# nanoporetech/pomfret

Measured on AMD Instinct MI355X. Metric: aligned reads/sec (methphase kernel), higher is better.
Workload: dtype u32/f32

## Files before the change

### pomfret_amd/csrc/pf_kernels.hip

```cpp
#include <hip/hip_runtime.h>
#include <stdint.h>
#include "pf_device.h"

#define DEV static __device__ __forceinline__

#ifdef PF_K3_PROFILE
DEV unsigned long long k3_stamp_now() {
    unsigned long long t;
    __builtin_amdgcn_sched_barrier(0);
    asm volatile("s_memtime %0\n\ts_waitcnt lgkmcnt(0)" : "=s"(t) :: "memory");
    __builtin_amdgcn_sched_barrier(0);
    return t;
}
#define K3_STAMP(i) do { const unsigned long long t_ = k3_stamp_now(); \
    prof_acc[i] += t_ - prof_last; prof_last = t_; } while (0)
DEV unsigned long long k3_realtime() {
    unsigned long long t;
    asm volatile("s_memrealtime %0\n\ts_waitcnt lgkmcnt(0)" : "=s"(t) :: "memory");
    return t;
}
#define K3_COUNT(i, v) do { prof_acc[i] += (v); } while (0)
#define K12_STAMP(i) do { if (threadIdx.x == 0) { const unsigned long long t_ = k3_stamp_now(); \
    d.prof[64ull * d.W + (uint64_t)w * 16 + (i)] = t_ - k12_t0; k12_t0 = t_; } } while (0)
#define K2_STAMP(i) do { if (k2acc) { const unsigned long long t_ = k3_stamp_now(); \
// ... 134 lines not shown
DEV double swap32_add_d(double x) {
    const long long b = __double_as_longlong(x);
    const auto lo = __builtin_amdgcn_permlane32_swap((uint32_t)b, (uint32_t)b, false, false);
    const auto hi = __builtin_amdgcn_permlane32_swap((uint32_t)(b >> 32), (uint32_t)(b >> 32), false, false);
    const double a = __longlong_as_double((long long)(((uint64_t)hi[0] << 32) | lo[0]));
    const double c = __longlong_as_double((long long)(((uint64_t)hi[1] << 32) | lo[1]));
    return a + c;
}
DEV double wave_group_sum_d(double x, uint32_t ncp) {
    if (ncp < 2) x = ror_add_d<1>(x);
    if (ncp < 4) x = ror_add_d<2>(x);
    if (ncp < 8) x = ror_add_d<4>(x);
    if (ncp < 16) x = ror_add_d<8>(x);
    if (ncp < 32) x = swap16_add_d(x);
    if (ncp < 64) x = swap32_add_d(x);
    return x;
}

DEV uint32_t rdl(uint32_t x, uint32_t l) { return (uint32_t)__builtin_amdgcn_readlane((int)x, (int)l); }

DEV uint64_t wave_max_u64(uint64_t x) {
#pragma unroll
    for (int o = 32; o > 0; o >>= 1) {
        uint64_t y = __shfl_xor(x, o, 64);
        x = y > x ? y : x;
    }
    return x;
}

template <int NT>
DEV uint32_t block_excl_scan(uint32_t v, uint32_t *sh, uint32_t *total) {
    const uint32_t tid = threadIdx.x, lane = tid & 63, wid = tid >> 6;
    constexpr int NW = NT / 64;
    uint32_t x = wave_incl_scan(v, lane);
    if (lane == 63) sh[wid] = x;
    __syncthreads();
    if (wid == 0) {
        uint32_t t = lane < (uint32_t)NW ? sh[lane] : 0;
        uint32_t s = wave_incl_scan(t, lane);
        if (lane < (uint32_t)NW) sh[lane] = s - t;
        if (lane == NW - 1) sh[NW] = s;
    }
    __syncthreads();
    uint32_t res = x - v + sh[wid];
    *total = sh[NW];
    __syncthreads();
    return res;
}

DEV uint64_t lb_u32(const uint32_t *a, uint64_t lo, uint64_t hi, uint32_t v) {
    while (lo < hi) {
        uint64_t mid = lo + ((hi - lo) >> 1);
        if (a[mid] < v) lo = mid + 1; else hi = mid;
    }
    return lo;
}
DEV uint64_t ub_u32(const uint32_t *a, uint64_t lo, uint64_t hi, uint32_t v) {
    while (lo < hi) {
        uint64_t mid = lo + ((hi - lo) >> 1);
        if (a[mid] <= v) lo = mid + 1; else hi = mid;
    }
    return lo;
}

DEV uint32_t next_pow2(uint32_t x) { return x <= 1 ? 1u : 1u << (32 - __clz(x - 1)); }


DEV void k2_chars(const pf_dev_batch &d, uint64_t c0, uint64_t c1, const uint32_t *sp, uint32_t qlo,
                  uint32_t qhi, uint32_t lane, uint8_t *chars) {
    const uint32_t nq = qhi - qlo;
    for (uint32_t j = lane; j < nq; j += 64) chars[j] = 2;
    wave_sync();
    const uint32_t plo = sp[qlo], phi = sp[qhi - 1];
    for (uint64_t cb = c0 + lane; cb < c1; cb += 256) {
        uint32_t pos[4], prv[4], cat[4];
#pragma unroll
        for (int u = 0; u < 4; u++) {
            const uint64_t c = cb + 64 * u;
            const bool ok = c < c1;
            pos[u] = ok ? d.call_pos[c] : 0xFFFFFFFFu;
            prv[u] = (ok && c > c0) ? d.call_pos[c - 1] : 0xFFFFFFFFu;
            cat[u] = ok ? d.call_cat[c] : 2u;
        }
#pragma unroll
        for (int u = 0; u < 4; u++) {
            const uint64_t c = cb + 64 * u;
            const uint32_t p = pos[u];
            if (c < c1 && (c == c0 || prv[u] != p) && p >= plo && p <= phi) {
                uint32_t lo = qlo, hi = qhi;
                while (lo < hi) {
                    const uint32_t mid = (lo + hi) >> 1;
                    if (sp[mid] < p) lo = mid + 1; else hi = mid;
                }
                if (lo < qhi && sp[lo] == p) chars[lo - qlo] = (uint8_t)cat[u];
            }
        }
    }
    wave_sync();
}

DEV void wave_lb2(const uint32_t *a, uint32_t n, uint32_t kA, uint32_t kB, uint32_t lane, uint32_t &lbA,
                  uint32_t &lbB) {
    const uint32_t h = lane >> 5, j = lane & 31;
    const uint32_t key = h ? kB : kA;
    uint32_t lo = 0, hi = n;
    for (;;) {
        const uint32_t len = hi - lo;
        const uint32_t step = (len + 31) >> 5;
        const uint32_t p = lo + j * step;
        const bool lt = len > 0 && p < hi && a[p] < key;
        const uint64_t bal = __ballot(lt);
        const uint32_t c = (uint32_t)__popc((uint32_t)(bal >> (32 * h)));
        if (len > 0) {
            if (c == 0) hi = lo;
            else {
                const uint32_t pn = lo + c * step;
                lo = lo + (c - 1) * step + 1;
                hi = pn < hi ? pn : hi;
            }
        }
        if (__ballot(hi > lo) == 0) break;
    }
    lbA = rdl(lo, 0);
    lbB = rdl(lo, 32);
}

struct K2SiteHash {
    const uint32_t *t;
    uint32_t mask, pmin;
};
DEV uint32_t k2_hash_slot(uint32_t rel) { return (rel * 2654435761u) >> 7; }
DEV uint32_t k2_site_of(const K2SiteHash &hs, uint32_t p) {
    const uint32_t rel = p - hs.pmin;
    if (p < hs.pmin || rel >= (1u << 19)) return PF_NONE;
    uint32_t h = k2_hash_slot(rel) & hs.mask;
    for (;;) {
        const uint32_t e = hs.t[h];
        if (e == PF_NONE) return PF_NONE;
        if ((e >> 13) == rel) return e & 8191u;
        h = (h + 1) & hs.mask;
    }
}

struct K2Read {
    uint64_t c0, c1;
    uint32_t F, L, cap, maxcall;
};

#define K2_CR 8
struct K2Calls {
    uint32_t pos[K2_CR], cat[K2_CR], site[K2_CR];
};

DEV void k2_calls_sites(K2Calls &cl, const uint32_t *sp, uint32_t S, const K2SiteHash hs, bool use_hash) {
#pragma unroll
    for (int u = 0; u < K2_CR; u++) {
        const uint32_t p = cl.pos[u];
        uint32_t si = PF_NONE;
        if (cl.cat[u] < 3u && S > 0 && p >= sp[0] && p <= sp[S - 1]) {
            if (use_hash) si = k2_site_of(hs, p);
            else {
                uint32_t lo = 0, hi = S;
                while (lo < hi) {
                    const uint32_t mid = (lo + hi) >> 1;
                    if (sp[mid] < p) lo = mid + 1; else hi = mid;
                }
                si = sp[lo] == p ? lo : PF_NONE;
            }
        }
        cl.site[u] = si;
    }
}

DEV void k2_load_scalars(const pf_dev_batch &d, uint32_t r, K2Read &rd) {
    rd.c0 = d.read_call_off[r];
    rd.c1 = d.read_call_end[r];
    rd.F = d.read_first[r];
    rd.L = d.read_last[r];
    rd.cap = d.mmr_cap[r];
    rd.maxcall = 0;
}

DEV void k2_issue_calls(const pf_dev_batch &d, const K2Read &rd, uint32_t lane, uint32_t *pos, uint32_t *cat) {
    const bool fits = rd.c1 - rd.c0 <= 64ull * K2_CR && rd.cap <= d.k12_capw;
#pragma unroll
    for (int u = 0; u < K2_CR; u++) {
        const uint64_t c = rd.c0 + lane + 64u * u;
        const bool ok = fits && c < rd.c1;
        pos[u] = ok ? d.call_pos[c] : 0xFFFFFFFFu;
        cat[u] = ok ? (uint32_t)d.call_cat[c] : 3u;
    }
}

DEV void k2_finish_calls(uint64_t c0, uint64_t c1, uint32_t lane, const uint32_t *pos, const uint32_t *cat,
                         K2Calls &cl) {
    uint32_t last = 0xFFFFFFFFu;
#pragma unroll
    for (int u = 0; u < K2_CR; u++) {
        const uint64_t c = c0 + lane + 64u * u;
        uint32_t prv = (uint32_t)__builtin_amdgcn_update_dpp(0, (int)pos[u], 0x138, 0xF, 0xF, false);
        if (lane == 0) prv = last;
        last = rdl(pos[u], 63);
        cl.pos[u] = pos[u];
        cl.cat[u] = (c < c1 && (c == c0 || prv != pos[u])) ? cat[u] : 3u;
    }
}

DEV void k2_chars_reg(const K2Calls &cl, uint32_t qlo, uint32_t qhi, uint32_t lane, uint8_t *chars) {
    const uint32_t nq = qhi - qlo;
    for (uint32_t j = lane; j < nq; j += 64) chars[j] = 2;
    wave_sync();
#pragma unroll
    for (int u = 0; u < K2_CR; u++) {
        const uint32_t si = cl.site[u];
        if (si >= qlo && si < qhi) chars[si - qlo] = (uint8_t)cl.cat[u];
    }
    wave_sync();
}

template <typename IR>
DEV uint32_t k2_core(const pf_dev_batch &d, uint32_t r, uint32_t dir, uint32_t lane, uint32_t S,
                     const uint32_t *sp, const uint32_t *st, const uint8_t *lens, const uint32_t *q1,
                     uint8_t *chars, uint8_t *crank, IR *irank, uint32_t capw, const K2Read &rd,
                     const K2Calls *cl, uint64_t koff, unsigned long long *k2acc = nullptr,
                     uint32_t *kst = nullptr) {
    uint32_t staged_n = 0;
    const uint32_t g = 2 * r + dir;
    const uint64_t c0 = rd.c0, c1 = rd.c1;
    uint32_t total = 0, start_i = PF_NONE;
    if (S > 0 && c1 > c0) {
        const uint32_t F = rd.F, L = rd.L;
        const uint32_t sfirst = st[0], slast = st[S - 1];
        if (!(F > slast || L < sfirst)) {
            uint32_t lbF, lbL;
            wave_lb2(st, S, F, L, lane, lbF, lbL);
            uint32_t xl, xr;
            if (F < sfirst) xl = 0;
            else xl = st[lbF] == F ? lbF : (lbF ? lbF - 1 : 0);
            xr = L > slast ? S : lbL;
            if (xl < xr) {
                const uint32_t qlo = dir ? q1[xl] : xl;
                const uint32_t qhi = dir ? q1[xr - 1] + 1 : xr;
                const uint32_t nq = qhi - qlo;
                const uint32_t cap = rd.cap;
                if (nq > capw || xr - xl > capw) {
                    if (lane == 0) atomicOr(d.status, PF_ST_INTERNAL);
                } else {
                    K2_STAMP(0);
                    if (cl) k2_chars_reg(*cl, qlo, qhi, lane, chars);
                    else k2_chars(d, c0, c1, sp, qlo, qhi, lane, chars);
                    K2_STAMP(1);
                    uint32_t E = 0;
                    for (uint32_t i0 = xl; i0 < xr; i0 += 64) {
                        const uint32_t i = i0 + lane;
                        bool ent = false;
                        if (i < xr) ent = !(i > 1 && st[i] == st[i - 1]);
                        const uint64_t m = __ballot(ent);
                        if (ent) {
                            const uint32_t rk = E + (uint32_t)__popcll(m & lanemask_lt(lane));
                            const uint32_t q = dir ? q1[i] : i;
                            crank[rk] = chars[q - qlo];
                            irank[rk] = (IR)i;
                        }
                        E += (uint32_t)__popcll(m);
                    }
                    wave_sync();
                    K2_STAMP(2);
                    if (E > 0) {
                        const uint32_t maxcall = rd.maxcall;
                        const uint32_t usable = E - (st[irank[E - 1]] > maxcall ? 1u : 0u);
                        if (lane == 0 && E >= 2 && irank[0] == 0 && irank[1] == 1 && st[1] == st[0])
                            crank[0] = 2;
                        wave_sync();
                        uint32_t *out = d.keys + koff;
                        const uint64_t room = d.keys_cap > koff ? d.keys_cap - koff : 0;
                        for (uint32_t e0 = 0; e0 < E; e0 += 64) {
                            const uint32_t e = e0 + lane;
                            uint32_t ne = 0, fj = PF_NONE, i = 0, P = 0;
                            if (e < E) {
                                i = irank[e];
                                P = st[i];
                                for (uint32_t j = i; j < S && st[j] == P; j++) {
                                    if (e + lens[j] <= usable) {
                                        if (fj == PF_NONE) fj = j;
                                        ne++;
                                    }
                                }
                            }
                            const uint32_t incl = wave_incl_scan_dpp(ne);
                            const uint32_t tot = rdl(incl, 63);
                            if (start_i == PF_NONE && tot > 0) {
                                const uint64_t m = __ballot(ne > 0);
                                const uint32_t src = (uint32_t)__ffsll((unsigned long long)m) - 1;
                                start_i = rdl(fj, src);
                            }
                            if (ne) {
                                uint32_t pos = total + incl - ne;
                                for (uint32_t j = i; j < S && st[j] == P; j++) {
                                    const uint32_t Lj = lens[j];
                                    if (e + Lj <= usable) {
                                        uint32_t key = 0;
                                        for (uint32_t t = 0; t < Lj; t++) key = key << 2 | crank[e + t];
                                        if (pos < cap && pos < room) {
                                            if (kst) kst[pos] = key;
                                            else out[pos] = key;
                                        }
                                        pos++;
                                    }
                                }
                            }
                            total += tot;
                        }
                        if (total > cap && lane == 0) atomicOr(d.status, PF_ST_KEYS_OVF);
                        staged_n = total < cap ? total : cap;
                        staged_n = staged_n < room ? staged_n : (uint32_t)room;
                        K2_STAMP(3);
                    }
                }
            }
        }
    }
    if (lane == 0) {
        d.mmr_n[g] = total;
        d.mmr_start[g] = total ? start_i : 0;
    }
    return staged_n;
}

DEV void k2_flush(const pf_dev_batch &d, const uint32_t *kst, uint64_t koff, uint32_t n, uint32_t lane) {
    uint32_t *out = d.keys + koff;
    for (uint32_t t = lane; t < n; t += 64) out[t] = kst[t];
}

__global__ __launch_bounds__(PF_K2_WAVES * 64) void pf_k2_methmers(pf_dev_batch d) {
    __shared__ uint8_t s_chars[PF_K2_WAVES][PF_K2_ENT_CAP];
    __shared__ uint8_t s_crank[PF_K2_WAVES][PF_K2_ENT_CAP];
    __shared__ uint32_t s_irank[PF_K2_WAVES][PF_K2_ENT_CAP];
    const uint32_t lane = threadIdx.x & 63, wid = threadIdx.x >> 6;
    const uint64_t n = 2ull * (*d.fb_ctr);
    for (uint64_t gw = (uint64_t)blockIdx.x * PF_K2_WAVES + wid; gw < n; gw += (uint64_t)gridDim.x * PF_K2_WAVES) {
        const uint32_t r = d.fb_list[gw >> 1], dir = (uint32_t)(gw & 1);
        const uint32_t w = d.read_win[r];
        const uint32_t S = d.win_S[w];
        const uint64_t sb = d.win_site_off[w];
        const uint32_t *sp = d.site_pos + sb;
        const uint32_t *st = dir ? d.st1_pos + sb : sp;
        const uint8_t *lens = (dir ? d.len1 : d.len0) + sb;
        const uint32_t *q1 = d.site_q1 + sb;
        const uint64_t bo = d.big_off[r];
        K2Read rd;
        rd.c0 = d.read_call_off[r];
        rd.c1 = d.read_call_end[r];
        rd.F = d.read_first[r];
        rd.L = d.read_last[r];
        rd.cap = d.mmr_cap[r];
        rd.maxcall = rd.c1 > rd.c0 ? d.call_pos[rd.c1 - 1] : 0u;
        const uint64_t koff = d.mmr_off[2ull * r + dir];
        if (bo == ~0ull) {
            k2_core(d, r, dir, lane, S, sp, st, lens, q1, s_chars[wid], s_crank[wid], s_irank[wid],
                    PF_K2_ENT_CAP, rd, nullptr, koff);
        } else {
            const uint32_t cap = d.mmr_cap[r];
            if (bo + 16ull * cap > d.big_cap) {
                if (lane == 0) { d.mmr_n[2 * r + dir] = 0; d.mmr_start[2 * r + dir] = 0; atomicOr(d.status, PF_ST_BIG_OVF); }
                continue;
            }
            uint8_t *b = d.big + bo + (dir ? 8ull * cap : 0);
            k2_core(d, r, dir, lane, S, sp, st, lens, q1, b, b + cap, reinterpret_cast<uint32_t *>(b + 4ull * cap),
                    cap, rd, nullptr, koff);
        }
    }
}

DEV void k12_methmers(const pf_dev_batch &d, uint32_t r0, uint32_t i0, uint32_t i1, uint32_t wid, uint32_t NW,
                      uint32_t lane, uint32_t S, const uint32_t *sp, const uint32_t *st1, const uint32_t *q1s,
                      const uint8_t *l0s, const uint8_t *l1s, const K2SiteHash &hsd, bool use_hash, uint8_t *wb,
                      unsigned long long *k2acc, uint32_t *rctr) {
        uint8_t *chars = wb, *crank = wb + PF_K12_CAPW;
        uint16_t *irank = reinterpret_cast<uint16_t *>(wb + 2 * PF_K12_CAPW);
        uint32_t *kst = reinterpret_cast<uint32_t *>(wb + 4 * PF_K12_CAPW);
        uint32_t pend_n = 0;
        uint64_t pend_off = 0;
        auto take = [&]() -> uint32_t {
            uint32_t v = 0;
            if (lane == 0) v = atomicAdd(rctr, 1u);
            return (uint32_t)__builtin_amdgcn_readfirstlane((int)v);
        };
        K2Read rdA, rdB;
        uint32_t pA[K2_CR], tA[K2_CR], pB[K2_CR], tB[K2_CR];
        const uint32_t iw = i0 + wid;
        uint32_t iB = iw < i1 ? take() : i1;
        if (iw < i1) k2_load_scalars(d, r0 + iw, rdA);
        if (iB < i1) k2_load_scalars(d, r0 + iB, rdB);
        k2_issue_calls(d, iw < i1 ? rdA : K2Read{0, 0, 0, 0, 0, 0}, lane, pA, tA);
        for (uint32_t i = iw; i < i1;) {
            const uint32_t r = r0 + i;
            K2_STAMP(6);
            K2Read rd = rdA;
            const uint64_t nc = rd.c1 - rd.c0;
            const bool regs = rd.cap <= d.k12_capw && nc <= 64ull * K2_CR;
            K2Calls cl;
            if (regs) {
                k2_finish_calls(rd.c0, rd.c1, lane, pA, tA, cl);
                uint32_t mc = 0;
                if (nc) {
                    const uint32_t ul = (uint32_t)((nc - 1) >> 6), ll = (uint32_t)((nc - 1) & 63);
#pragma unroll
                    for (int u = 0; u < K2_CR; u++)
                        if ((uint32_t)u == ul) mc = rdl(cl.pos[u], ll);
                }
                rd.maxcall = mc;
                k2_calls_sites(cl, sp, S, hsd, use_hash);
            }
            K2_STAMP(4);
            k2_flush(d, kst, pend_off, pend_n, lane);
            pend_n = 0;
            K2Read rdC = {0, 0, 0, 0, 0, 0};
            const uint32_t iC = iB < i1 ? take() : i1;
            if (iC < i1) k2_load_scalars(d, r0 + iC, rdC);
            k2_issue_calls(d, iB < i1 ? rdB : K2Read{0, 0, 0, 0, 0, 0}, lane, pB, tB);
            K2_STAMP(8);
            if (rd.cap > d.k12_capw) {
                if (lane == 0) d.fb_list[atomicAdd(d.fb_ctr, 1u)] = r;
            } else {
                const uint64_t k0 = d.mmr_off[2ull * r], k1 = d.mmr_off[2ull * r + 1];
                if (regs) {
                    const uint32_t n0 = k2_core(d, r, 0, lane, S, sp, sp, l0s, q1s, chars, crank, irank, PF_K12_CAPW,
                                                rd, &cl, k0, k2acc, kst);
                    k2_flush(d, kst, k0, n0, lane);
                    K2_STAMP(5);
                    pend_n = k2_core(d, r, 1, lane, S, sp, st1, l1s, q1s, chars, crank, irank, PF_K12_CAPW, rd,
                                     &cl, k1, k2acc, kst);
                    pend_off = k1;
                    K2_STAMP(5);
                } else {
                    rd.maxcall = nc ? d.call_pos[rd.c1 - 1] : 0u;
                    k2_core(d, r, 0, lane, S, sp, sp, l0s, q1s, chars, crank, irank, PF_K12_CAPW, rd, nullptr, k0);
                    k2_core(d, r, 1, lane, S, sp, st1, l1s, q1s, chars, crank, irank, PF_K12_CAPW, rd, nullptr, k1);
                }
            }
            rdA = rdB;
            rdB = rdC;
            i = iB;
            iB = iC;
#pragma unroll
            for (int u = 0; u < K2_CR; u++) { pA[u] = pB[u]; tA[u] = tB[u]; }
            K2_STAMP(7);
        }
        k2_flush(d, kst, pend_off, pend_n, lane);
}

#ifndef PF_K12_CU
#define PF_K12_CU 4
#endif
template <typename F>
DEV void k12_each_call(const pf_dev_batch &d, uint32_t r0, uint32_t R, uint32_t wid, uint32_t NW, uint32_t lane,
                       F &&f) {
    constexpr uint32_t U = PF_K12_CU;
    const uint32_t wu = (uint32_t)__builtin_amdgcn_readfirstlane((int)wid);
    for (uint32_t ib = wu; ib < R; ib += 64 * NW) {
        const uint32_t i = ib + lane * NW;
        uint32_t blo = 0, bhi = 0, n = 0;
        if (i < R) {
            const uint64_t b = d.read_call_off[r0 + i];
            blo = (uint32_t)b;
            bhi = (uint32_t)(b >> 32);
            n = (uint32_t)(d.read_call_end[r0 + i] - b);
        }
        const uint32_t cnt = min(64u, (R - ib + NW - 1) / NW);
        auto range = [&](uint32_t j, uint64_t &b, uint32_t &m) {
            const uint32_t jj = min(j, 63u);
            b = ((uint64_t)rdl(bhi, jj) << 32) | rdl(blo, jj);
            m = j < cnt ? rdl(n, jj) : 0u;
        };
        uint32_t j = 0, o = 0, cn, nn;
        uint64_t cb, nb;
        range(0, cb, cn);
        range(1, nb, nn);
        while (j < cnt) {
            uint64_t c[U];
            bool ok[U];
#pragma unroll
            for (uint32_t u = 0; u < U; u++) {
                const uint32_t rem = cn - o;
                const bool cur = lane < rem;
                const uint32_t l2 = lane - rem;
                ok[u] = cur || l2 < nn;
                c[u] = !ok[u] ? 0ull : cur ? cb + o + lane : nb + l2;
                if (rem > 64) {
                    o += 64;
                } else {
                    o = min(64u - rem, nn);
                    j++;
                    cb = nb;
                    cn = nn;
                    range(j + 1, nb, nn);
                }
            }
            uint32_t cat[U], pos[U];
#pragma unroll
            for (uint32_t u = 0; u < U; u++) {
                cat[u] = d.call_cat[c[u]];
                pos[u] = d.call_pos[c[u]];
            }
#pragma unroll
            for (uint32_t u = 0; u < U; u++) f(ok[u] ? cat[u] : 2u, pos[u]);
        }
    }
}

__device__ __forceinline__ uint32_t mask_lower(const uint32_t *p, uint32_t lo, uint32_t hi, uint32_t x) {
    while (lo < hi) {
        const uint32_t mid = lo + ((hi - lo) >> 1);
        if (p[mid] < x) lo = mid + 1;
        else hi = mid;
    }
    return lo;
}

__global__ __launch_bounds__(PF_K1_THREADS) void pf_k12_sites_methmers(pf_dev_batch d) {
    __shared__ uint32_t tile[PF_K1_TILE];
    __shared__ uint32_t sh_scan[PF_K1_THREADS / 64 + 1];
    __shared__ uint32_t sh_misc[8];
    __shared__ unsigned long long sh_base[2];
    constexpr uint32_t NT = PF_K1_THREADS, NW = NT / 64;
    const uint32_t w = d.k12_order[blockIdx.x], tid = threadIdx.x, lane = tid & 63, wid = tid >> 6;
#ifdef PF_K3_PROFILE
    unsigned long long k12_t0 = __builtin_amdgcn_s_memtime();
#endif
    const uint32_t r0 = d.win_read_off[w], R = d.win_read_off[w + 1] - r0;
    const int cov = d.win_par[w * 4 + 0];
    const uint32_t s = d.win_start[w];
    const uint64_t sb = d.win_site_off[w];
    const uint32_t scap = d.win_site_cap[w];

    if (tid < 8) sh_misc[tid] = 0;
    __syncthreads();
    if (tid == 0) { sh_misc[2] = 0xFFFFFFFFu; sh_misc[3] = 0; }
    __syncthreads();
    for (uint32_t i = tid; i < R; i += NT) {
        const uint32_t r = r0 + i;
        if (d.read_start[r] <= s) {
            const uint32_t hp = d.read_hp[r];
            if (hp < 2) atomicAdd(&sh_misc[hp], 1u);
        }
        const uint64_t c0 = d.read_call_off[r], c1 = d.read_call_end[r];
        if (c1 > c0) {
            atomicMin(&sh_misc[2], d.call_pos[c0]);
            atomicMax(&sh_misc[3], d.call_pos[c1 - 1]);
            atomicAdd(&sh_misc[7], (uint32_t)(c1 - c0));
        }
    }
    __syncthreads();
    const bool fail = R == 0 || (int)sh_misc[0] < d.hard_cov || (int)sh_misc[1] < d.hard_cov ||
                      sh_misc[2] > sh_misc[3];
    if (fail) {
        if (tid == 0) { d.win_S[w] = 0; d.win_nreads[w] = 0; d.win_masked[w] = 0; }
        for (uint32_t i = tid; i < R; i += NT) {
            const uint32_t r = r0 + i;
            d.mmr_n[2 * r] = 0; d.mmr_n[2 * r + 1] = 0;
            d.mmr_start[2 * r] = 0; d.mmr_start[2 * r + 1] = 0;
            d.mmr_off[2 * r] = 0; d.mmr_off[2 * r + 1] = 0;
            d.mmr_cap[r] = 0;
            d.big_off[r] = ~0ull;
        }
        return;
    }
    K12_STAMP(1);
    const uint32_t pmin = sh_misc[2], pmax = sh_misc[3];
    uint32_t mk0 = 0, mk1 = 0;
    if (d.mask_n != 0) {
        const uint32_t a = d.win_mask_rng ? d.win_mask_rng[2 * w] : 0u;
        const uint32_t b = d.win_mask_rng ? d.win_mask_rng[2 * w + 1] : d.mask_n;
        mk0 = mask_lower(d.mask_pos, a, b, pmin);
        mk1 = mask_lower(d.mask_pos, mk0, b, pmax + 1);
    }
    if (tid == 0) { sh_misc[4] = 0; d.win_nreads[w] = R; }
    __syncthreads();

    constexpr uint32_t BW = 8192, RMAX = 12288, SEGB = BW * 64, MAXSEG = 2;
    static_assert(BW / 2 + RMAX <= PF_K1_TILE / 2, "word ranks + counters fit the first half of the tile");
    uint64_t *bmap = reinterpret_cast<uint64_t *>(tile + PF_K1_TILE / 2);
    const uint32_t nseg = d.k12_dense ? 0u : (uint32_t)min<uint64_t>(((uint64_t)(pmax - pmin) + SEGB) / SEGB, MAXSEG + 1);
    const bool range_ok = nseg >= 1 && nseg <= MAXSEG;
    bool fast = range_ok;
// ... 278 lines not shown
                const uint64_t ki = ((uint64_t)d.read_end[r0 + i]) << 32 | i;
                uint32_t rank = 0;
                for (uint32_t j = 0; j < R; j++) rank += (((uint64_t)d.read_end[r0 + j]) << 32 | j) < ki;
                d.rev_ord[r0 + rank] = i;
            }
        }
    }

    K12_STAMP(3);
    __syncthreads();
    const bool staged = S <= d.k12_smax;
    uint32_t *sp = tile, *st1 = tile + S, *q1s = tile + 2 * S;
    uint8_t *l0s = reinterpret_cast<uint8_t *>(tile + 3 * S), *l1s = l0s + S;
    const uint32_t *a = staged ? sp : d.site_pos + sb;
    if (staged) {
        for (uint32_t p = tid; p < S; p += NT) sp[p] = d.site_pos[sb + p];
        __syncthreads();
    }
    const uint32_t k = (uint32_t)d.k, span = (uint32_t)d.k_span;
    for (uint32_t p = tid; p < S; p += NT) {
        const uint32_t ap = a[p];
        uint32_t j = p + k > S - 1 ? S - 1 : p + k;
        while (a[j] - ap > span) j--;
        const uint8_t v0 = (uint8_t)(j == p ? 1 : j - p);
        uint32_t q = p > k ? p - k : 0;
        while (ap - a[q] > span) q++;
        const uint8_t v1 = (uint8_t)(q == p ? 1 : p - q);
        const uint32_t s1 = a[q];
        d.len0[sb + p] = v0;
        d.len1[sb + p] = v1;
        d.st1_pos[sb + p] = s1;
        d.site_q1[sb + p] = q;
        if (staged) { l0s[p] = v0; l1s[p] = v1; st1[p] = s1; q1s[p] = q; }
    }
    K12_STAMP(4);
    uint32_t tot_keys = 0, tot_big = 0;
    for (uint32_t i0 = 0; i0 < R; i0 += NT) {
        const uint32_t i = i0 + tid;
        uint32_t bound = 0, bigb = 0;
        if (i < R) {
            const uint32_t r = r0 + i;
            const uint64_t c0 = d.read_call_off[r], c1 = d.read_call_end[r];
            if (c1 > c0 && S > 0) {
                const uint32_t F = d.read_first[r], L = d.read_last[r];
                const uint64_t lbF = lb_u32(a, 0, S, F), ubL = ub_u32(a, 0, S, L);
                const uint32_t cnt = ubL > lbF ? (uint32_t)(ubL - lbF) : 0;
                bound = cnt + 3 * k + 4;
                if (bound > d.k2_entcap) bigb = 16 * bound;
            }
            d.mmr_cap[r] = bound;
        }
        uint32_t t1, t2;
        block_excl_scan<NT>(bound, sh_scan, &t1);
        block_excl_scan<NT>(bigb, sh_scan, &t2);
        tot_keys += t1;
        tot_big += t2;
    }
    if (tid == 0) {
        const unsigned long long kb = atomicAdd(d.keys_ctr, 2ull * tot_keys);
        if (kb + 2ull * tot_keys > d.keys_cap) atomicOr(d.status, PF_ST_KEYS_OVF);
        sh_base[0] = kb;
        unsigned long long bb = 0;
        if (tot_big) {
            bb = atomicAdd(d.big_ctr, (unsigned long long)tot_big);
            if (bb + tot_big > d.big_cap) atomicOr(d.status, PF_ST_BIG_OVF);
        }
        sh_base[1] = bb;
    }
    __syncthreads();
    if (sh_base[0] + 2ull * tot_keys > d.keys_cap) {
        for (uint32_t i = tid; i < R; i += NT) {
            const uint32_t r = r0 + i;
            d.mmr_n[2 * r] = 0; d.mmr_n[2 * r + 1] = 0;
            d.mmr_start[2 * r] = 0; d.mmr_start[2 * r + 1] = 0;
            d.mmr_off[2 * r] = 0; d.mmr_off[2 * r + 1] = 0;
            d.big_off[r] = ~0ull;
        }
        if (tid == 0) d.win_S[w] = 0;
        return;
    }
    uint64_t kcarry = sh_base[0], bcarry = sh_base[1];
    for (uint32_t i0 = 0; i0 < R; i0 += NT) {
        const uint32_t i = i0 + tid;
        uint32_t bound = 0, bigb = 0;
        if (i < R) {
            bound = d.mmr_cap[r0 + i];
            if (bound > d.k2_entcap) bigb = 16 * bound;
        }
        uint32_t t1, t2;
        const uint32_t e1 = block_excl_scan<NT>(bound, sh_scan, &t1);
        const uint32_t e2 = block_excl_scan<NT>(bigb, sh_scan, &t2);
        if (i < R) {
            const uint32_t r = r0 + i;
            d.mmr_off[2 * r] = kcarry + 2ull * e1;
            d.mmr_off[2 * r + 1] = kcarry + 2ull * e1 + bound;
            d.big_off[r] = bigb ? bcarry + e2 : ~0ull;
        }
        kcarry += 2ull * t1;
        bcarry += t2;
    }

    K12_STAMP(5);
    const uint32_t arr_b = (uint32_t)((14ull * S + 15) & ~15ull);
    uint32_t HS = 1;
    while (HS < S * 4) HS <<= 1;
    const bool use_hash = staged && fast && nseg == 1 && arr_b + 4u * HS + 16u * PF_K12_WB * PF_K12_CAPW <= 4u * PF_K1_TILE;
    uint32_t *hst = reinterpret_cast<uint32_t *>(reinterpret_cast<uint8_t *>(tile) + arr_b);
    if (tid == 0) sh_misc[5] = NW;
    if (use_hash) {
        for (uint32_t j = tid; j < HS; j += NT) hst[j] = PF_NONE;
        __syncthreads();
        for (uint32_t p = tid; p < S; p += NT) {
            const uint32_t rel = sp[p] - pmin;
            uint32_t h = k2_hash_slot(rel) & (HS - 1);
            while (atomicCAS(&hst[h], PF_NONE, (rel << 13) | p) != PF_NONE) h = (h + 1) & (HS - 1);
        }
    }
    __syncthreads();
    K2SiteHash hsd;
    hsd.t = hst;
    hsd.mask = HS - 1;
    hsd.pmin = pmin;

    if (staged && R >= d.k12c_minr && S <= d.k12c_smax) {
        for (uint32_t c = tid; c * PF_K12C_READS < R; c += NT) {
            const uint32_t k = atomicAdd(d.k12c_ctr, 1u);
            d.k12c_list[2ull * k] = w;
            d.k12c_list[2ull * k + 1] = c * PF_K12C_READS;
        }
    } else if (staged) {
        uint8_t *wb = reinterpret_cast<uint8_t *>(tile) + arr_b + (use_hash ? 4u * HS : 0u) +
                      wid * (uint64_t)PF_K12_WB * PF_K12_CAPW;
#ifdef PF_K3_PROFILE
        unsigned long long k2a[10] = {0, 0, 0, 0, 0, 0, 0, 0, 0, __builtin_amdgcn_s_memtime()};
        unsigned long long *k2acc = wid == 0 ? k2a : nullptr;
#else
        unsigned long long *k2acc = nullptr;
#endif
        k12_methmers(d, r0, 0, R, wid, NW, lane, S, sp, st1, q1s, l0s, l1s, hsd, use_hash, wb, k2acc, &sh_misc[5]);
#ifdef PF_K3_PROFILE
        if (tid == 0) {
            for (int j = 0; j < 7; j++) d.prof[64ull * d.W + (uint64_t)w * 16 + 8 + j] = k2a[j];
            d.prof[64ull * d.W + (uint64_t)w * 16 + 7] = k2a[7];
            d.prof[64ull * d.W + (uint64_t)w * 16 + 15] = k2a[8];
        }
#endif
    } else {
        for (uint32_t i = tid; i < R; i += NT) d.fb_list[atomicAdd(d.fb_ctr, 1u)] = r0 + i;
    }
    __syncthreads();
    K12_STAMP(6);
}

__global__ __launch_bounds__(PF_K12C_WAVES * 64) void pf_k12_chunks(pf_dev_batch d) {
    extern __shared__ __attribute__((aligned(16))) uint8_t smem[];
    __shared__ uint32_t s_item, s_rctr;
    const uint32_t tid = threadIdx.x, lane = tid & 63u, wid = tid >> 6;
    const uint32_t n = *d.k12c_ctr;
    for (;;) {
        if (tid == 0) s_item = atomicAdd(d.k12c_next, 1u);
        __syncthreads();
        const uint32_t it = s_item;
        if (it >= n) break;
        const uint32_t w = d.k12c_list[2ull * it], c0 = d.k12c_list[2ull * it + 1];
        if (tid == 0) s_rctr = c0 + PF_K12C_WAVES;
        const uint32_t r0 = d.win_read_off[w], R = d.win_read_off[w + 1] - r0;
        const uint32_t S = d.win_S[w];
        const uint64_t sb = d.win_site_off[w];
        uint32_t *sp = reinterpret_cast<uint32_t *>(smem), *st1 = sp + S, *q1s = sp + 2 * S;
        uint8_t *l0s = reinterpret_cast<uint8_t *>(sp + 3 * S), *l1s = l0s + S;
        for (uint32_t p = tid; p < S; p += PF_K12C_WAVES * 64) {
            sp[p] = d.site_pos[sb + p];
            st1[p] = d.st1_pos[sb + p];
            q1s[p] = d.site_q1[sb + p];
            l0s[p] = d.len0[sb + p];
            l1s[p] = d.len1[sb + p];
        }
        __syncthreads();
        const uint32_t arr_b = (uint32_t)((14ull * S + 15) & ~15ull);
        uint8_t *wb = smem + arr_b + wid * (uint64_t)PF_K12_WB * PF_K12_CAPW;
        K2SiteHash hsd;
        hsd.t = nullptr; hsd.mask = 0; hsd.pmin = 0;
        const uint32_t c1 = min(R, c0 + PF_K12C_READS);
        k12_methmers(d, r0, c0, c1, wid, PF_K12C_WAVES, lane, S, sp, st1, q1s, l0s, l1s, hsd, false, wb, nullptr,
                     &s_rctr);
        __syncthreads();
    }
}

struct K3Ctl {
    uint32_t S, R, ntot, nc, L, done, failed, inserted, winner, tag;
    int32_t i_last;
    uint32_t min_i, max_i, fail, summ, nstrict, mxlen, cmax;
    uint32_t path, need, cacheb;
    unsigned long long t_run;
    uint32_t ins_n, ins_st, ins_mo, ins_tg;
    unsigned long long scr;
    int32_t tab[4];
};

struct K3Cand {
    uint32_t read[PF_MAX_NCAND];
    uint32_t pos[PF_MAX_NCAND];
    uint32_t site0[PF_MAX_NCAND];
    uint32_t len[PF_MAX_NCAND];
    uint32_t kofs[PF_MAX_NCAND];
    unsigned long long key[PF_MAX_NCAND];
    uint8_t tag[PF_MAX_NCAND];
};

template <int NTH>
struct K3CandSlimT {
    uint32_t read[NTH];
    uint32_t pos[128];
    unsigned long long key[256];
};
using K3CandSlim = K3CandSlimT<PF_K3S_THREADS>;

DEV uint64_t align16(uint64_t x) { return (x + 15) & ~15ull; }

template <int NT, typename K, typename F>
DEV void k3_each_key(const pf_dev_batch &d, uint32_t r0, uint32_t R, uint32_t dir, K &&keep, F &&f) {
    constexpr uint32_t B = 8, NW = NT / 64;
    const uint32_t lane = threadIdx.x & 63, wid = threadIdx.x >> 6;
    for (uint32_t i0 = wid * B; i0 < R; i0 += NW * B) {
        uint32_t n[B], st[B], key[B];
        uint64_t off[B];
#pragma unroll
        for (uint32_t u = 0; u < B; u++) {
            const uint32_t i = i0 + u;
            const bool ok = i < R && keep(i);
            const uint64_t g = 2ull * (r0 + (ok ? i : 0u)) + dir;
            n[u] = ok ? d.mmr_n[g] : 0u;
            st[u] = d.mmr_start[g];
            off[u] = d.mmr_off[g];
        }
#pragma unroll
        for (uint32_t u = 0; u < B; u++) key[u] = lane < n[u] ? d.keys[off[u] + lane] : 0u;
#pragma unroll
        for (uint32_t u = 0; u < B; u++)
            if (lane < n[u]) f(i0 + u, lane, st[u] + lane, off[u] + lane, key[u]);
#pragma unroll
        for (uint32_t u = 0; u < B; u++)
            for (uint32_t t = 64 + lane; t < n[u]; t += 64) f(i0 + u, t, st[u] + t, off[u] + t, d.keys[off[u] + t]);
    }
}

template <int NT = PF_K3_THREADS>
DEV void k3_dict(const pf_dev_batch &d, uint32_t r0, uint32_t R, uint32_t S, uint32_t dir,
                 uint64_t *masks, uint32_t *base, uint32_t *sh_scan, K3Ctl &ctl) {
    const uint32_t tid = threadIdx.x;
    const uint32_t MW = (uint32_t)d.mw;
    for (uint32_t j = tid; j < S * MW; j += NT) masks[j] = 0;
    __syncthreads();
    k3_each_key<NT>(d, r0, R, dir, [](uint32_t) { return true; },
                    [&](uint32_t, uint32_t, uint32_t site, uint64_t, uint32_t key) {
                        if (site < S && key < 64u * MW)
                            atomicOr((unsigned long long *)&masks[(uint64_t)site * MW + (key >> 6)], 1ull << (key & 63));
                    });
    __syncthreads();
    uint32_t carry = 0;
    for (uint32_t p0 = 0; p0 < S; p0 += NT) {
        const uint32_t p = p0 + tid;
        uint32_t c = 0;
        if (p < S)
            for (uint32_t m = 0; m < MW; m++) c += (uint32_t)__popcll(masks[(uint64_t)p * MW + m]);
        uint32_t tot;
        const uint32_t ex = block_excl_scan<NT>(c, sh_scan, &tot);
        if (p < S) base[p] = carry + ex;
        carry += tot;
    }
    if (tid == 0) ctl.ntot = carry;
    __syncthreads();
}

template <int NT = PF_K3_THREADS>
DEV void k3_dict_rewrite(const pf_dev_batch &d, uint32_t r0, uint32_t R, uint32_t S, uint32_t dir,
                         const uint64_t *masks, const uint32_t *base) {
    const uint32_t MW = (uint32_t)d.mw;
    k3_each_key<NT>(d, r0, R, dir, [](uint32_t) { return true; },
                    [&](uint32_t, uint32_t, uint32_t site, uint64_t koff, uint32_t key) {
                        uint32_t slot = PF_NONE;
                        if (site < S && key < 64u * MW) {
                            const uint64_t *row = masks + (uint64_t)site * MW;
                            const uint32_t wi = key >> 6, b = key & 63;
                            slot = base[site];
                            for (uint32_t m = 0; m < wi; m++) slot += (uint32_t)__popcll(row[m]);
                            slot += (uint32_t)__popcll(row[wi] & ((1ull << b) - 1ull));
                        }
                        d.keys[koff] = slot;
                    });
    __syncthreads();
}

DEV uint32_t kd_hash(uint32_t key) {
    const uint32_t h = key * 0x9E3779B1u;
    return h ^ (h >> 15);
}
DEV void kd_sync() {
    __builtin_amdgcn_fence(__ATOMIC_RELEASE, "agent");
    __syncthreads();
    __builtin_amdgcn_fence(__ATOMIC_ACQUIRE, "agent");
}

__global__ __launch_bounds__(PF_K3_THREADS) void pf_k3_kdict(pf_dev_batch d) {
    constexpr uint32_t NT = PF_K3_THREADS, NW = NT / 64;
    __shared__ uint32_t sh_scan[NW + 1];
    __shared__ unsigned long long s_o;
    __shared__ uint32_t s_fail;
    const uint32_t prob = blockIdx.x, w = prob >> 1, dir = prob & 1;
// ... 2666 lines not shown
```

Measured before the change: 56.30 million.

## Add paired forward/reverse methmer extraction with packed 2-bit key windows

Adds a k2_pair path that computes both strands' site ranges in one wave-cooperative 16-way lower-bound search, loads call characters once, and builds keys from 2-bit packed words instead of looping over bytes. It falls back to the two separate k2_core passes when the ranges do not fit. It also skips site lookup for call slots beyond the call count, marks the wave id as uniform, and pins pf_k12_chunks to 4 waves per EU. The goal is to cut duplicated searches and per-byte key assembly, at the cost of more code and register pressure and a possible occupancy limit.

```diff
diff --git a/pomfret_amd/csrc/pf_kernels.hip b/pomfret_amd/csrc/pf_kernels.hip
--- a/pomfret_amd/csrc/pf_kernels.hip
+++ b/pomfret_amd/csrc/pf_kernels.hip
@@ -310,12 +310,15 @@
     uint32_t pos[K2_CR], cat[K2_CR], site[K2_CR];
 };
 
-DEV void k2_calls_sites(K2Calls &cl, const uint32_t *sp, uint32_t S, const K2SiteHash hs, bool use_hash) {
+DEV void k2_calls_sites(K2Calls &cl, uint32_t nc, const uint32_t *sp, uint32_t S, const K2SiteHash hs,
+                        bool use_hash) {
+    const uint32_t sfirst = S ? sp[0] : 1u, slast = S ? sp[S - 1] : 0u;
 #pragma unroll
     for (int u = 0; u < K2_CR; u++) {
         const uint32_t p = cl.pos[u];
         uint32_t si = PF_NONE;
-        if (cl.cat[u] < 3u && S > 0 && p >= sp[0] && p <= sp[S - 1]) {
+        if (64u * u >= nc) { cl.site[u] = si; continue; }
+        if (cl.cat[u] < 3u && p >= sfirst && p <= slast) {
             if (use_hash) si = k2_site_of(hs, p);
             else {
                 uint32_t lo = 0, hi = S;
@@ -530,6 +533,261 @@
     }
 }
 
+#ifndef PF_K12_PAIR
+#define PF_K12_PAIR 1
+#endif
+#ifndef PF_K12_PACK
+#define PF_K12_PACK 1
+#endif
+
+DEV void wave_lb4(const uint32_t *a0, const uint32_t *a1, uint32_t n, uint32_t kA, uint32_t kB, uint32_t lane,
+                  uint32_t &lbA0, uint32_t &lbB0, uint32_t &lbA1, uint32_t &lbB1) {
+    const uint32_t g = lane >> 4, j = lane & 15;
+    const uint32_t *a = a0 + ((g & 2u) ? (a1 - a0) : 0);
+    const uint32_t key = (g & 1u) ? kB : kA;
+    uint32_t lo = 0, hi = n;
+    for (;;) {
+        const uint32_t len = hi - lo;
+        const uint32_t step = (len + 15) >> 4;
+        const uint32_t p = lo + j * step;
+        const bool lt = len > 0 && p < hi && a[p] < key;
+        const uint64_t bal = __ballot(lt);
+        const uint32_t c = (uint32_t)__popc((uint32_t)(bal >> (16 * g)) & 0xFFFFu);
+        if (len > 0) {
+            if (c == 0) hi = lo;
+            else {
+                const uint32_t pn = lo + c * step;
+                lo = lo + (c - 1) * step + 1;
+                hi = pn < hi ? pn : hi;
+            }
+        }
+        if (__ballot(hi > lo) == 0) break;
+    }
+    lbA0 = rdl(lo, 0);
+    lbB0 = rdl(lo, 16);
+    lbA1 = rdl(lo, 32);
+    lbB1 = rdl(lo, 48);
+}
+
+DEV void k2_pack_chars(const uint8_t *cb, uint32_t n, uint32_t lane, uint32_t *pk) {
+    const uint32_t *c4 = reinterpret_cast<const uint32_t *>(cb);
+    for (uint32_t w = lane; 16 * w < n; w += 64) {
+        uint32_t v = 0;
+#pragma unroll
+        for (int q = 0; q < 4; q++) {
+            const uint32_t t = c4[4 * w + q] & 0x03030303u;
+            v = v << 8 | (t * 0x40100401u) >> 24;
+        }
+        pk[w] = v;
+    }
+}
+DEV uint64_t k2_key_window(const uint32_t *pk, uint32_t e) {
+    const uint32_t w = e >> 4;
+    return (uint64_t)pk[w] << 32 | pk[w + 1];
+}
+DEV uint32_t k2_key_of(uint64_t win, uint32_t e, uint32_t L) {
+    return L ? (uint32_t)((win << (2 * (e & 15u))) >> ((64 - 2 * L) & 63u)) : 0u;
+}
+DEV uint32_t k2_key_bytes(const uint8_t *cb, uint32_t e, uint32_t L) {
+    uint32_t key = 0;
+    for (uint32_t t = 0; t < L; t++) key = key << 2 | cb[e + t];
+    return key;
+}
+
+DEV bool k2_pair(const pf_dev_batch &d, uint32_t r, uint32_t lane, uint32_t S, const uint32_t *sp,
+                 const uint32_t *st1, const uint32_t *q1s, const uint8_t *l0s, const uint8_t *l1s, uint8_t *wb,
+                 const K2Read &rd, const K2Calls &cl, uint64_t k0, uint64_t k1, unsigned long long *k2acc,
+                 uint32_t &pend_n) {
+    uint8_t *chars = wb, *crank = wb + PF_K12_CAPW;
+    uint16_t *irank = reinterpret_cast<uint16_t *>(wb + 2 * PF_K12_CAPW);
+    uint32_t *kst = reinterpret_cast<uint32_t *>(wb + 4 * PF_K12_CAPW);
+    uint32_t *pk0 = reinterpret_cast<uint32_t *>(crank), *pk1 = reinterpret_cast<uint32_t *>(chars);
+    (void)pk0; (void)pk1;
+    pend_n = 0;
+    uint32_t xl0 = 0, xr0 = 0, xl1 = 0, xr1 = 0;
+    if (S > 0 && rd.c1 > rd.c0) {
+        const uint32_t F = rd.F, L = rd.L;
+        const uint32_t sf0 = sp[0], sl0 = sp[S - 1], sf1 = st1[0], sl1 = st1[S - 1];
+        const bool in0 = !(F > sl0 || L < sf0), in1 = !(F > sl1 || L < sf1);
+        if (in0 || in1) {
+            uint32_t lbF0, lbL0, lbF1, lbL1;
+            wave_lb4(sp, st1, S, F, L, lane, lbF0, lbL0, lbF1, lbL1);
+            if (in0) {
+                xl0 = F < sf0 ? 0 : (sp[lbF0] == F ? lbF0 : (lbF0 ? lbF0 - 1 : 0));
+                xr0 = L > sl0 ? S : lbL0;
+            }
+            if (in1) {
+                xl1 = F < sf1 ? 0 : (st1[lbF1] == F ? lbF1 : (lbF1 ? lbF1 - 1 : 0));
+                xr1 = L > sl1 ? S : lbL1;
+            }
+        }
+    }
+    const bool ne0 = xl0 < xr0, ne1 = xl1 < xr1;
+    if (ne0 != ne1) return false;
+    if (!ne0) {
+        if (lane == 0) {
+            d.mmr_n[2 * r] = 0; d.mmr_start[2 * r] = 0;
+            d.mmr_n[2 * r + 1] = 0; d.mmr_start[2 * r + 1] = 0;
+        }
+        return true;
+    }
+    const uint32_t ql1 = q1s[xl1], qh1 = q1s[xr1 - 1] + 1;
+    const uint32_t ulo = xl0 < ql1 ? xl0 : ql1, uhi = xr0 > qh1 ? xr0 : qh1;
+    if (xr0 - xl0 > PF_K12_CAPW || xr1 - xl1 > PF_K12_CAPW || uhi - ulo > d.k12_capw) return false;
+    K2_STAMP(0);
+    k2_chars_reg(cl, ulo, uhi, lane, chars);
+    const uint32_t cap = rd.cap, maxcall = rd.maxcall;
+    {
+        const uint32_t E = xr0 - xl0, off = xl0 - ulo;
+        const uint32_t usable = E - (sp[xr0 - 1] > maxcall ? 1u : 0u);
+#if PF_K12_PACK
+        k2_pack_chars(chars, uhi - ulo, lane, pk0);
+        wave_sync();
+#endif
+        K2_STAMP(1);
+        const uint64_t room = d.keys_cap > k0 ? d.keys_cap - k0 : 0;
+        uint32_t total = 0, start_i = PF_NONE;
+        for (uint32_t e0 = 0; e0 < E; e0 += 64) {
+            const uint32_t e = e0 + lane;
+            bool emit = false;
+            uint32_t key = 0;
+            if (e < E) {
+                const uint32_t Lj = l0s[xl0 + e];
+#if PF_K12_PACK
+                const uint64_t win = k2_key_window(pk0, off + e);
+#endif
+                emit = e + Lj <= usable;
+#if PF_K12_PACK
+                key = k2_key_of(win, off + e, Lj);
+#else
+                if (emit) key = k2_key_bytes(chars, off + e, Lj);
+#endif
+            }
+            const uint64_t m = __ballot(emit);
+            if (start_i == PF_NONE && m) start_i = xl0 + e0 + (uint32_t)__ffsll((unsigned long long)m) - 1;
+            if (emit) {
+                const uint32_t pos = total + (uint32_t)__popcll(m & lanemask_lt(lane));
+                if (pos < cap && pos < room) kst[pos] = key;
+            }
+            total += (uint32_t)__popcll(m);
+        }
+        if (total > cap && lane == 0) atomicOr(d.status, PF_ST_KEYS_OVF);
+        uint32_t n0 = total < cap ? total : cap;
+        n0 = n0 < room ? n0 : (uint32_t)room;
+        K2_STAMP(3);
+        if (lane == 0) {
+            d.mmr_n[2 * r] = total;
+            d.mmr_start[2 * r] = total ? start_i : 0;
+        }
+        k2_flush(d, kst, k0, n0, lane);
+        K2_STAMP(5);
+    }
+    {
+        const uint32_t qlo = ulo;
+        uint32_t E = 0;
+        for (uint32_t i0 = xl1; i0 < xr1; i0 += 64) {
+            const uint32_t i = i0 + lane;
+            bool ent = false;
+            if (i < xr1) ent = !(i > 1 && st1[i] == st1[i - 1]);
+            const uint64_t m = __ballot(ent);
+            if (ent) {
+                const uint32_t rk = E + (uint32_t)__popcll(m & lanemask_lt(lane));
+                crank[rk] = chars[q1s[i] - qlo];
+                irank[rk] = (uint16_t)i;
+            }
+            E += (uint32_t)__popcll(m);
+        }
+        wave_sync();
+        uint32_t total = 0, start_i = PF_NONE, n1 = 0;
+        if (E > 0) {
+            const uint32_t usable = E - (st1[irank[E - 1]] > maxcall ? 1u : 0u);
+            const bool dup01 = xl1 == 0 && xr1 >= 2 && st1[1] == st1[0];
+#if PF_K12_PACK
+            k2_pack_chars(crank, E, lane, pk1);
+            if (dup01 && lane == 0) pk1[0] = (pk1[0] & 0x3FFFFFFFu) | 0x80000000u;
+            wave_sync();
+#else
+            if (dup01 && lane == 0) crank[0] = 2;
+            wave_sync();
+#endif
+            K2_STAMP(2);
+            const uint64_t room = d.keys_cap > k1 ? d.keys_cap - k1 : 0;
+            for (uint32_t e0 = 0; e0 < E; e0 += 64) {
+                const uint32_t e = e0 + lane;
+                uint32_t ne = 0, fj = PF_NONE, i = 0, P = 0;
+                uint64_t lp = 0;
+#if PF_K12_PACK
+                uint64_t win = 0;
+#endif
+                if (e < E) {
+                    i = irank[e];
+#if PF_K12_PACK
+                    win = k2_key_window(pk1, e);
+#endif
+                    P = st1[i];
+                    uint32_t j = i;
+                    bool more;
+                    do {
+                        const uint32_t Lj = l1s[j];
+                        more = j + 1 < S && st1[j + 1] == P;
+                        if (e + Lj <= usable) {
+                            if (fj == PF_NONE) fj = j;
+                            if (ne < 8) lp |= (uint64_t)Lj << (8 * ne);
+                            ne++;
+                        }
+                        j++;
+                    } while (more);
+                }
+                const uint32_t incl = wave_incl_scan_dpp(ne);
+                const uint32_t tot = rdl(incl, 63);
+                if (start_i == PF_NONE && tot > 0) {
+                    const uint64_t m = __ballot(ne > 0);
+                    const uint32_t src = (uint32_t)__ffsll((unsigned long long)m) - 1;
+                    start_i = rdl(fj, src);
+                }
+                if (ne) {
+                    uint32_t pos = total + incl - ne;
+                    if (ne <= 8) {
+                        for (uint32_t t = 0; t < ne; t++, pos++) {
+                            const uint32_t Lj = (uint32_t)(lp >> (8 * t)) & 255u;
+#if PF_K12_PACK
+                            const uint32_t key = k2_key_of(win, e, Lj);
+#else
+                            const uint32_t key = k2_key_bytes(crank, e, Lj);
+#endif
+                            if (pos < cap && pos < room) kst[pos] = key;
+                        }
+                    } else {
+                        for (uint32_t j = i; j < S && st1[j] == P; j++) {
+                            const uint32_t Lj = l1s[j];
+                            if (e + Lj <= usable) {
+#if PF_K12_PACK
+                                const uint32_t key = k2_key_of(win, e, Lj);
+#else
+                                const uint32_t key = k2_key_bytes(crank, e, Lj);
+#endif
+                                if (pos < cap && pos < room) kst[pos] = key;
+                                pos++;
+                            }
+                        }
+                    }
+                }
+                total += tot;
+            }
+            if (total > cap && lane == 0) atomicOr(d.status, PF_ST_KEYS_OVF);
+            n1 = total < cap ? total : cap;
+            n1 = n1 < room ? n1 : (uint32_t)room;
+            K2_STAMP(3);
+        }
+        if (lane == 0) {
+            d.mmr_n[2 * r + 1] = total;
+            d.mmr_start[2 * r + 1] = total ? start_i : 0;
+        }
+        pend_n = n1;
+    }
+    return true;
+}
+
 DEV void k12_methmers(const pf_dev_batch &d, uint32_t r0, uint32_t i0, uint32_t i1, uint32_t wid, uint32_t NW,
                       uint32_t lane, uint32_t S, const uint32_t *sp, const uint32_t *st1, const uint32_t *q1s,
                       const uint8_t *l0s, const uint8_t *l1s, const K2SiteHash &hsd, bool use_hash, uint8_t *wb,
@@ -568,7 +826,7 @@
                         if ((uint32_t)u == ul) mc = rdl(cl.pos[u], ll);
                 }
                 rd.maxcall = mc;
-                k2_calls_sites(cl, sp, S, hsd, use_hash);
+                k2_calls_sites(cl, uni((uint32_t)nc), sp, S, hsd, use_hash);
             }
             K2_STAMP(4);
             k2_flush(d, kst, pend_off, pend_n, lane);
@@ -583,12 +841,19 @@
             } else {
                 const uint64_t k0 = d.mmr_off[2ull * r], k1 = d.mmr_off[2ull * r + 1];
                 if (regs) {
-                    const uint32_t n0 = k2_core(d, r, 0, lane, S, sp, sp, l0s, q1s, chars, crank, irank, PF_K12_CAPW,
-                                                rd, &cl, k0, k2acc, kst);
-                    k2_flush(d, kst, k0, n0, lane);
-                    K2_STAMP(5);
-                    pend_n = k2_core(d, r, 1, lane, S, sp, st1, l1s, q1s, chars, crank, irank, PF_K12_CAPW, rd,
-                                     &cl, k1, k2acc, kst);
+#if PF_K12_PAIR
+                    const bool paired = k2_pair(d, r, lane, S, sp, st1, q1s, l0s, l1s, wb, rd, cl, k0, k1, k2acc, pend_n);
+#else
+                    const bool paired = false;
+#endif
+                    if (!paired) {
+                        const uint32_t n0 = k2_core(d, r, 0, lane, S, sp, sp, l0s, q1s, chars, crank, irank,
+                                                    PF_K12_CAPW, rd, &cl, k0, k2acc, kst);
+                        k2_flush(d, kst, k0, n0, lane);
+                        K2_STAMP(5);
+                        pend_n = k2_core(d, r, 1, lane, S, sp, st1, l1s, q1s, chars, crank, irank, PF_K12_CAPW, rd,
+                                         &cl, k1, k2acc, kst);
+                    }
                     pend_off = k1;
                     K2_STAMP(5);
                 } else {
@@ -1173,10 +1438,10 @@
     K12_STAMP(6);
 }
 
-__global__ __launch_bounds__(PF_K12C_WAVES * 64) void pf_k12_chunks(pf_dev_batch d) {
+__global__ __launch_bounds__(PF_K12C_WAVES * 64) __attribute__((amdgpu_waves_per_eu(4, 4))) void pf_k12_chunks(pf_dev_batch d) {
     extern __shared__ __attribute__((aligned(16))) uint8_t smem[];
     __shared__ uint32_t s_item, s_rctr;
-    const uint32_t tid = threadIdx.x, lane = tid & 63u, wid = tid >> 6;
+    const uint32_t tid = threadIdx.x, lane = tid & 63u, wid = uni(tid >> 6);
     const uint32_t n = *d.k12c_ctr;
     for (;;) {
         if (tid == 0) s_item = atomicAdd(d.k12c_next, 1u);
```

Result: faster. 57.30 million (median of 6 runs) (+1.8%).
